# afermg/aliby

Measured on AMD Instinct MI355X. Metric: FOV tiles/sec (whole node), higher is better.
Workload: dtype u16 pixels, f64 feature accumulators, f32 dynamics, bfloat16 U-Net

## Files before the change

aliby_amd/csrc/nn_conv.hip:

```cpp
#include "common.h"
#include "conv_launch.h"
#include "conv_mfma.h"

namespace {

struct ConvArgs {
  const uint4* in;
  const uint4* wpk;
  uint4* out;
  uint4* pool;
  const float* scale;
  const float* shift;
  const float* bias;
  const uint4* res;
  int shift_stride, res_up;
  int cs, coff;
  int ocs, ocoff;
  int N, H, W;
  int G;
  int tiles_x, tiles_y, ntiles;
  int order;
  const uint4* pin;
  const uint4* pwpk;
  int pcs;
// ... 430 lines not shown
    if constexpr (PACK) {
      g0 = (tx * TW) / a.W;
      cst = tx * TW - g0 * a.W;
      half = (a.W - cst) >> 1;
    }
    const uint4* inN = a.in + (size_t)(PACK ? n * a.G : n) * IH * IW * a.cs + a.coff;
    int t0 = tid;
    asm volatile("" : "+v"(t0));
#pragma unroll
    for (int k = 0; k < GIT; ++k) {
      const int unit = t0 + k * 256;
      const int rpix = unit / NPL, oct = unit % NPL;
      const int rly = rpix / RLW, rlx = rpix - rly * RLW;
      const int iy = min(max(ry0 + rly, 0), IH - 1);
      int ix, img = 0;
      if constexpr (PACK) {
        const bool first = rlx <= half;
        ix = min(max(first ? (cst >> 1) - 1 + rlx : rlx - half - 1, 0), IW - 1);
        img = first ? g0 : min(g0 + 1, a.G - 1);
      } else {
        ix = min(max(rx0 + rlx, 0), IW - 1);
      }
      const uint4* g = inN + (unsigned)(((img * IH + iy) * IW + ix) * a.cs + oct);
      __builtin_amdgcn_global_load_lds((const __attribute__((address_space(1))) void*)g,
                                       (__attribute__((address_space(3))) void*)(ldsR + k * 256 + wave_u * 64), 16, 0, 0);
    }
  };

  if (walk.count > 0) issue_dma(walk.first);
  for (int stamp_tile = 0; stamp_tile < walk.count; ++stamp_tile) {
    const int tile = walk.first + stamp_tile * walk.step;
    CONV_STAMP(0);
    const int tx = tile % a.tiles_x, tyn = tile / a.tiles_x;
    const int ty = tyn % a.tiles_y, n = tyn / a.tiles_y;
    const int y0 = ty * TH, x0 = tx * TW;
    int g0 = 0, cst = x0, kb = 1 << 20, nimg = n;
    if constexpr (PACK) {
      g0 = x0 / a.W;
      cst = x0 - g0 * a.W;
      kb = a.W - cst;
      nimg = n * a.G;
    }
    const int second = (PACK && px >= kb) ? 1 : 0;
    const int gx = PACK ? (second ? px - kb : cst + px) : x0 + px;
    const int irow = PACK ? (g0 + second) * a.H : 0;

    f32x2_t sh[4], sh1[PACK ? 4 : 1];
    {
      const float* sp = a.shift + (size_t)(nimg + g0) * a.shift_stride + pl * 8;
#pragma unroll
      for (int k = 0; k < 4; ++k) sh[k] = f32x2_t{sp[2 * k], sp[2 * k + 1]};
      if constexpr (PACK) {
        const float* sq = a.shift + (size_t)(nimg + min(g0 + 1, a.G - 1)) * a.shift_stride + pl * 8;
#pragma unroll
        for (int k = 0; k < 4; ++k) sh1[k] = f32x2_t{sq[2 * k], sq[2 * k + 1]};
      }
    }
    float4 b4[4] = {};
    if (a.bias) {
      const float4* bp = reinterpret_cast<const float4*>(a.bias + c0);
#pragma unroll
      for (int q = 0; q < 4; ++q) b4[q] = bp[q];
    }
    uint4 rr[R][2];
    auto load_res = [&](int pass) { conv_load_res<R>(a, nimg, irow, y0 + (rg * PASSES + pass) * R, gx, c0, rr); };
    if (a.res) load_res(0);
    CONV_STAMP(1);
    asm volatile("s_waitcnt vmcnt(0)" ::: "memory");
    __syncthreads();
    CONV_STAMP(2);
    if constexpr (cfg::LOWA) {
      const int ry0 = (y0 >> 1) - 1, rx0 = (x0 >> 1) - 1;
      int p0 = pix0;
      asm volatile("" : "+v"(p0));
#pragma unroll
      for (int it = 0; it < ITERS; ++it) {
        const int rpix = p0 + it * PIX_PER_IT;
        const int rly = rpix / RLW, rlx = rpix - rly * RLW;
        const unsigned keep = 0u - (unsigned)((unsigned)(ry0 + rly) < (unsigned)IH && (unsigned)(rx0 + rlx) < (unsigned)IW);
        const uint4 o = conv_act8(ldsR[min(rpix, cfg::APIX - 1) * NPL + pl], sc, sh, keep);
        if (it == ITERS - 1 && rpix >= cfg::APIX) continue;
        ldsA[pl * PLANE + rpix] = o;
      }
    } else {
      const int ry0 = UP ? (y0 >> 1) - 1 : y0 - 1, rx0 = UP ? (x0 >> 1) - 1 : x0 - 1;
      int p0 = pix0, qy = ly0, qx = lx0;
      asm volatile("" : "+v"(p0), "+v"(qy), "+v"(qx));
#pragma unroll
      for (int it = 0; it < ITERS; ++it) {
        int lx = qx + (it * PIX_PER_IT) % LW, ly = qy + (it * PIX_PER_IT) / LW;
        if (lx >= LW) { lx -= LW; ly += 1; }
        const int gy = y0 - 1 + ly, gxi = x0 - 1 + lx;
        const int pix = p0 + it * PIX_PER_IT;
        unsigned keep;
        int rpix;
        uint4 o;
        if constexpr (PACK) {
          const int gapi = kb < 32 ? kb + 1 : TW + 2;
          const int bp = lx - 1 - (lx > gapi ? 1 : 0);
          const int snd = bp >= kb ? 1 : 0;
          const int c = snd ? bp - kb : cst + bp;
          keep = 0u - (unsigned)(lx != gapi && c >= 0 && c < a.W && !(bp == TW && kb == TW) && (unsigned)gy < (unsigned)a.H);
          const int rcol = snd ? (kb >> 1) + 1 + (c >> 1) : ((cst + bp) >> 1) - ((cst >> 1) - 1);
          rpix = min(max(((gy >> 1) - ry0) * RLW + rcol, 0), cfg::RLH * RLW - 1);
          f32x2_t shs[4];
#pragma unroll
          for (int k = 0; k < 4; ++k) shs[k] = snd ? sh1[k] : sh[k];
          o = conv_act8(ldsR[rpix * NPL + pl], sc, shs, keep);
        } else {
          keep = 0u - (unsigned)((unsigned)gy < (unsigned)a.H && (unsigned)gxi < (unsigned)a.W);
          rpix = UP ? min(((gy >> 1) - ry0) * RLW + ((gxi >> 1) - rx0), cfg::RLH * RLW - 1) : min(pix, RAW - 1);
          o = conv_act8(ldsR[rpix * NPL + pl], sc, sh, keep);
        }
        if (it == ITERS - 1 && pix >= RAW) continue;
        ldsA[pl * PLANE + pix] = o;
      }
    }
    CONV_STAMP(3);
    __syncthreads();
#pragma unroll
    for (int pass = 0; pass < PASSES; ++pass) {
      const int rbase = (rg * PASSES + pass) * R;
      f32x16_t acc[R];
      conv_seed<R>(acc, b4, rr, a.res != nullptr);
      __builtin_amdgcn_sched_barrier(0);
      if (pass == 0 && stamp_tile + 1 < walk.count) issue_dma(tile + walk.step);
      if (pass + 1 < PASSES && a.res) load_res(pass + 1);
      __builtin_amdgcn_sched_barrier(0);
      if (pass == 0) CONV_STAMP(4);
      if constexpr (cfg::LOWA) {
        const bf16x8_t* L0 = reinterpret_cast<const bf16x8_t*>(ldsA) + hh * PLANE + (rbase >> 1) * RLW + ((px + 1) >> 1);
        conv_mfma<R, KC, cfg::DEPTH, PLANE, RLW, true>(L0, wfrag, acc, L0 + 1 - (px & 1));
      } else {
        conv_mfma<R, KC, cfg::DEPTH, PLANE, LW>(reinterpret_cast<const bf16x8_t*>(ldsA) + hh * PLANE + rbase * LW + px + second, wfrag, acc);
      }
      if (pass == PASSES - 1) CONV_STAMP(5);
      conv_store<R>(a, nimg, irow, y0 + rbase, gx, c0, acc);
    }
    CONV_STAMP(6);
  }
}

struct PairBase {
  static constexpr int KC = 2, NPL = 4, R = 2, PASSES = 2;
  static constexpr int TH = 14, TWO = 30, MH = 16, MW = 32;
  static constexpr int RAW_MID = MH * MW, PLANE_MID = RAW_MID + (10 - RAW_MID % 8) % 8;
  static constexpr int MID_SLOTS = NPL * PLANE_MID + 8;
  static constexpr int DEPTH = 6;
};
struct PairCfg : PairBase {
  static constexpr int IH = 18, IW = 34;
  static constexpr int RAW_IN = IH * IW, PLANE_IN = RAW_IN + (10 - RAW_IN % 8) % 8;
  static constexpr int PIX_PER_IT = 256 / NPL, ITERS = (RAW_IN + PIX_PER_IT - 1) / PIX_PER_IT;
  static constexpr int SLOTS = NPL * PLANE_IN + 2 * MID_SLOTS;
  static constexpr int LDS_BYTES = SLOTS * 16;
};

template <bool POOL, bool HEAD>
__global__ __launch_bounds__(512, 1) void k_conv_pair32(ConvArgs a) {
  static_assert(!(POOL && HEAD), "either the pooled output (down block) or the output head (last unit)");
  using cfg = PairCfg;
  constexpr int KC = cfg::KC, NPL = cfg::NPL, R = cfg::R, PASSES = cfg::PASSES, TH = cfg::TH, TWO = cfg::TWO;
  constexpr int IW_ = cfg::IW, MW = cfg::MW, PLANE_IN = cfg::PLANE_IN, PLANE_MID = cfg::PLANE_MID, RAW_IN = cfg::RAW_IN;
  constexpr int PIX_PER_IT = cfg::PIX_PER_IT, ITERS = cfg::ITERS;
  extern __shared__ uint4 lds[];
  uint4* const ldsIn = lds;
  uint4* const ldsMid0 = lds + NPL * PLANE_IN;
  __shared__ __align__(16) float tabB[64];
  __shared__ __align__(16) float biasA[32];
  __shared__ float hconst[HEAD ? 2 * 32 + 4 : 1];

  const int consumer = threadIdx.x >> 8;
  const int tid = threadIdx.x & 255, lane = tid & 63, wave = tid >> 6;
  const int px = lane & 31, hh = lane >> 5;
  const int c0 = hh * 16;

  const TileWalk walk = tile_walk(a.ntiles, a.order);
  const int my_tiles = walk.count;

  if (!consumer) {
    bf16x8_t wA[9 * KC];
    {
      const bf16x8_t* pa = reinterpret_cast<const bf16x8_t*>(a.wpk) + lane;
#pragma unroll
      for (int i = 0; i < 9 * KC; ++i) wA[i] = pa[i * 64];
    }
    const int pl = tid % NPL, pix0 = tid / NPL;
    const int ly0 = pix0 / IW_, lx0 = pix0 - ly0 * IW_;
    f32x2_t sc[4];
#pragma unroll
    for (int k = 0; k < 4; ++k) sc[k] = f32x2_t{a.scale[pl * 8 + 2 * k], a.scale[pl * 8 + 2 * k + 1]};
    if (tid < 32) biasA[tid] = a.bias ? a.bias[tid] : 0.f;
    uint4 v[ITERS];
    unsigned inside = 0;
    auto request = [&](int tile) {
      const int tx = tile % a.tiles_x, tyn = tile / a.tiles_x;
      const int ty = tyn % a.tiles_y, n = tyn / a.tiles_y;
      const int y0 = ty * TH, x0 = tx * TWO;
      const uint4* inN = a.in + (size_t)n * a.H * a.W * a.cs + a.coff;
      inside = 0;
#pragma unroll
      for (int u = 0; u < ITERS; ++u) {
        int lx = lx0 + (u * PIX_PER_IT) % IW_, ly = ly0 + (u * PIX_PER_IT) / IW_;
        if (lx >= IW_) { lx -= IW_; ly += 1; }
        const int gy = y0 - 2 + ly, gxi = x0 - 2 + lx;
        inside |= (unsigned)((unsigned)gy < (unsigned)a.H && (unsigned)gxi < (unsigned)a.W) << u;
        const int cy = min(max(gy, 0), a.H - 1), cx = min(max(gxi, 0), a.W - 1);
        v[u] = inN[(unsigned)((cy * a.W + cx) * a.cs + pl)];
      }
    };
    if (my_tiles > 0) request(walk.first);
    for (int it = 0; it < my_tiles; ++it) {
      const int tile = walk.first + it * walk.step;
      const int tx = tile % a.tiles_x, tyn = tile / a.tiles_x;
      const int ty = tyn % a.tiles_y, n = tyn / a.tiles_y;
      const int y0 = ty * TH, x0 = tx * TWO;
      uint4* const ldsMid = ldsMid0 + (it & 1) * cfg::MID_SLOTS;
      f32x2_t sh[4];
      {
        const float* sp = a.shift + (size_t)n * a.shift_stride + pl * 8;
#pragma unroll
        for (int k = 0; k < 4; ++k) sh[k] = f32x2_t{sp[2 * k], sp[2 * k + 1]};
      }
      if (tid < 32) {
        tabB[tid] = a.scale2[tid];
        tabB[32 + tid] = a.shift2[(size_t)n * a.shift2_stride + tid];
      }
#pragma unroll
      for (int u = 0; u < ITERS; ++u) {
        const uint4 o = conv_act8(v[u], sc, sh, 0u - ((inside >> u) & 1u));
        if (u == ITERS - 1 && pix0 + u * PIX_PER_IT >= RAW_IN) continue;
        ldsIn[pl * PLANE_IN + pix0 + u * PIX_PER_IT] = o;
      }
      __syncthreads();
      if (it + 1 < my_tiles) request(tile + walk.step);
      __builtin_amdgcn_sched_barrier(0);
#pragma unroll
      for (int pass = 0; pass < PASSES; ++pass) {
        const int mbase = (wave * PASSES + pass) * R;
        f32x16_t acc[R];
        {
          float4 b4[4];
#pragma unroll
          for (int q = 0; q < 4; ++q) b4[q] = reinterpret_cast<const float4*>(biasA + c0)[q];
#pragma unroll
          for (int r = 0; r < R; ++r) acc_seed(acc[r], b4);
        }
        __builtin_amdgcn_sched_barrier(0);
        conv_mfma<R, KC, cfg::DEPTH, PLANE_IN, IW_>(reinterpret_cast<const bf16x8_t*>(ldsIn) + hh * PLANE_IN + mbase * IW_ + px, wA, acc);
        __builtin_amdgcn_sched_barrier(0);
        const int mgx = x0 - 1 + px;
#pragma unroll
        for (int r = 0; r < R; ++r) {
          const int mgy = y0 - 1 + mbase + r;
          const unsigned keep = 0u - (unsigned)((unsigned)mgy < (unsigned)a.H && (unsigned)mgx < (unsigned)a.W);
#pragma unroll
          for (int half = 0; half < 2; ++half) {
            f32x2_t s2[4], h2[4];
            const float4* tp = reinterpret_cast<const float4*>(tabB + c0 + 8 * half);
            const float4 sa = tp[0], sb = tp[1], ha = tp[8], hb = tp[9];
            s2[0] = f32x2_t{sa.x, sa.y}; s2[1] = f32x2_t{sa.z, sa.w}; s2[2] = f32x2_t{sb.x, sb.y}; s2[3] = f32x2_t{sb.z, sb.w};
            h2[0] = f32x2_t{ha.x, ha.y}; h2[1] = f32x2_t{ha.z, ha.w}; h2[2] = f32x2_t{hb.x, hb.y}; h2[3] = f32x2_t{hb.z, hb.w};
            const uint4 raw = make_uint4(cv_pack2(acc[r][8 * half + 0], acc[r][8 * half + 1]), cv_pack2(acc[r][8 * half + 2], acc[r][8 * half + 3]),
                                         cv_pack2(acc[r][8 * half + 4], acc[r][8 * half + 5]), cv_pack2(acc[r][8 * half + 6], acc[r][8 * half + 7]));
            ldsMid[(2 * hh + half) * PLANE_MID + (mbase + r) * MW + px] = conv_act8(raw, s2, h2, keep);
          }
        }
      }
      __syncthreads();
    }
    __syncthreads();
    __syncthreads();
  } else {
    bf16x8_t wB[9 * KC];
    {
      const bf16x8_t* pb = reinterpret_cast<const bf16x8_t*>(a.wpk2) + lane;
#pragma unroll
      for (int i = 0; i < 9 * KC; ++i) wB[i] = pb[i * 64];
    }
    HeadW hwf;
    if constexpr (HEAD) {
      hwf = head_weights(a.hw, a.hO, lane);
      if (tid < 32) {
        hconst[tid] = a.hscale[tid];
        hconst[32 + tid] = a.hshift[tid];
        if (tid < 4) hconst[64 + tid] = tid < a.hO ? a.hbias[tid] : 0.f;
      }
    }
    float4 b4[4];
    load_bias4(a.bias2, c0, b4);
    __syncthreads();
    __syncthreads();
    for (int it = 0; it < my_tiles; ++it) {
      const int tile = walk.first + it * walk.step;
      const int tx = tile % a.tiles_x, tyn = tile / a.tiles_x;
      const int ty = tyn % a.tiles_y, n = tyn / a.tiles_y;
      const int y0 = ty * TH, x0 = tx * TWO;
      const uint4* const ldsMid = ldsMid0 + (it & 1) * cfg::MID_SLOTS;
      const int gx = (px < TWO && x0 + px < a.W) ? x0 + px : a.W;
#pragma unroll
      for (int pass = 0; pass < PASSES; ++pass) {
        const int rbase = (wave * PASSES + pass) * R;
        if (rbase < TH) {
          uint4 rr[R][2];
          if (a.res) conv_load_res<R>(a, n, 0, y0 + rbase, min(gx, a.W - 1), c0, rr);
          f32x16_t acc[R];
          conv_seed<R>(acc, b4, rr, a.res != nullptr);
          __builtin_amdgcn_sched_barrier(0);
          conv_mfma<R, KC, cfg::DEPTH, PLANE_MID, MW>(reinterpret_cast<const bf16x8_t*>(ldsMid) + hh * PLANE_MID + rbase * MW + px, wB, acc);
          if constexpr (HEAD) {
#pragma unroll
            for (int r = 0; r < R; ++r) {
              const f32x16_t y = head_from_acc(acc[r], hconst, hconst + 32, hwf, hh);
              const int gy = y0 + rbase + r;
              if (hh == 0 && gx < a.W && gy < a.H) {
                float* hp = a.hout + (size_t)n * a.hO * a.H * a.W + (size_t)gy * a.W + gx;
                const float yo[4] = {y[0], y[1], y[2], y[3]};
                for (int o = 0; o < a.hO; ++o) hp[(size_t)o * a.H * a.W] = yo[o] + hconst[64 + o];
              }
            }
          }
          if (!HEAD || a.out) conv_store<R>(a, n, 0, y0 + rbase, gx, c0, acc);
          if constexpr (POOL) {
            const int PH = a.H >> 1, PW = a.W >> 1;
            const int gy = y0 + rbase;
            const bool writer = (px & 1) == 0 && gx + 1 < a.W && gy + 1 < a.H;
            uint4* pp = a.pool + (size_t)n * PH * PW * a.ocs + a.ocoff + (unsigned)(((gy >> 1) * PW + (min(gx, a.W - 1) >> 1)) * a.ocs + (c0 >> 3));
#pragma unroll
            for (int half = 0; half < 2; ++half) {
              unsigned pk[4];
#pragma unroll
              for (int q = 0; q < 4; ++q) {
                const float v0 = fmaxf(acc[0][half * 8 + 2 * q], acc[1][half * 8 + 2 * q]);
                const float v1 = fmaxf(acc[0][half * 8 + 2 * q + 1], acc[1][half * 8 + 2 * q + 1]);
                pk[q] = cv_pack2(fmaxf(v0, __shfl_xor(v0, 1)), fmaxf(v1, __shfl_xor(v1, 1)));
              }
              if (writer) pp[half] = make_uint4(pk[0], pk[1], pk[2], pk[3]);
            }
          }
        }
        __syncthreads();
      }
    }
  }
}

struct FirstPairCfg : PairBase {
  static constexpr int AH = 18, AW = 36;
  static constexpr int P0_WORDS = 2 * AH * AW;
  static constexpr int RAWP_WORDS = MH * MW;
  static constexpr int VALS = 2 * AH * AW, ITERS = (VALS + 255) / 256;
  static constexpr int LDS_BYTES = 2 * MID_SLOTS * 16 + P0_WORDS * 4 + 2 * RAWP_WORDS * 4;
};

__global__ __launch_bounds__(512, 1) void k_conv_first_pair(ConvArgs a) {
  using cfg = FirstPairCfg;
  constexpr int KC = cfg::KC, R = cfg::R, PASSES = cfg::PASSES, TH = cfg::TH, TWO = cfg::TWO, MW = cfg::MW;
  constexpr int AH = cfg::AH, AW = cfg::AW, PLANE_MID = cfg::PLANE_MID, ITERS = cfg::ITERS;
  extern __shared__ uint4 lds[];
  uint4* const ldsMid0 = lds;
  unsigned* const P0 = reinterpret_cast<unsigned*>(lds + 2 * cfg::MID_SLOTS);
  unsigned* const rawP0 = P0 + cfg::P0_WORDS;
  __shared__ __align__(16) float tabB[64];

  const int consumer = threadIdx.x >> 8;
  const int tid = threadIdx.x & 255, lane = tid & 63, wave = tid >> 6;
  const int px = lane & 31, hh = lane >> 5;
  const int c0 = hh * 16;

  const TileWalk walk = tile_walk(a.ntiles, a.order);
  const int my_tiles = walk.count;
  const size_t plane = (size_t)a.H * a.W;

  if (!consumer) {
    bf16x8_t wF[2];
    {
      const int m = lane & 31, co = conv_row_channel(m);
#pragma unroll
      for (int kc = 0; kc < 2; ++kc) {
        unsigned r4[4];
#pragma unroll
        for (int j2 = 0; j2 < 4; ++j2) {
          float v[2];
#pragma unroll
          for (int e = 0; e < 2; ++e) {
            const int k = 16 * kc + 8 * hh + 2 * j2 + e, c = k / 12, ty = (k % 12) / 4, tx = k % 4;
            v[e] = (c < a.fcin && tx < 3 && k < 24) ? a.fw[((size_t)co * a.fcin + c) * 9 + ty * 3 + tx] : 0.f;
          }
          r4[j2] = cv_pack2(v[0], v[1]);
        }
        wF[kc] = __builtin_bit_cast(bf16x8_t, make_uint4(r4[0], r4[1], r4[2], r4[3]));
      }
    }
    int goff[2][2];
    unsigned gmask[2][2];
#pragma unroll
    for (int kc = 0; kc < 2; ++kc)
#pragma unroll
      for (int g = 0; g < 2; ++g) {
        const int k = 16 * kc + 8 * hh + 4 * g;
        const bool live = k < 24 && k / 12 < a.fcin;
        goff[kc][g] = live ? (k / 12) * AH * AW + ((k % 12) / 4) * AW : 0;
        gmask[kc][g] = live ? 0xffffffffu : 0u;
      }
    if (tid < 32) {
      tabB[tid] = a.scale2[tid];
      tabB[32 + tid] = a.shift2[tid];
    }
    const float fs0 = a.fscale[0], fh0 = a.fshift[0];
    const float fs1 = a.fcin > 1 ? a.fscale[1] : 0.f, fh1 = a.fcin > 1 ? a.fshift[1] : 0.f;
    float v[ITERS];
    unsigned inside = 0;
    auto request = [&](int tile) {
      const int tx = tile % a.tiles_x, tyn = tile / a.tiles_x;
      const int ty = tyn % a.tiles_y, n = tyn / a.tiles_y;
      const int y0 = ty * TH, x0 = tx * TWO;
      inside = 0;
#pragma unroll
      for (int u = 0; u < ITERS; ++u) {
        const int i = tid + 256 * u;
        const int c = i / (AH * AW), rem = i - c * (AH * AW), r = rem / AW, q = rem - r * AW;
        const int gy = y0 - 2 + r, gx = x0 - 2 + q;
        const bool ok = i < cfg::VALS && c < a.fcin && (unsigned)gy < (unsigned)a.H && (unsigned)gx < (unsigned)a.W;
        inside |= (unsigned)ok << u;
        const int cy = min(max(gy, 0), a.H - 1), cx = min(max(gx, 0), a.W - 1), cc = min(c, a.fcin - 1);
        v[u] = a.fx[((size_t)n * a.fcin + cc) * plane + (size_t)cy * a.W + cx];
      }
    };
    if (my_tiles > 0) request(walk.first);
    unsigned short* const P0h = reinterpret_cast<unsigned short*>(P0);
    for (int it = 0; it < my_tiles; ++it) {
      const int tile = walk.first + it * walk.step;
      const int tx = tile % a.tiles_x, tyn = tile / a.tiles_x;
      const int ty = tyn % a.tiles_y;
      const int y0 = ty * TH, x0 = tx * TWO;
      uint4* const ldsMid = ldsMid0 + (it & 1) * cfg::MID_SLOTS;
      unsigned short* const rawPh = reinterpret_cast<unsigned short*>(rawP0 + (it & 1) * cfg::RAWP_WORDS);
#pragma unroll
      for (int u = 0; u < ITERS; ++u) {
        const int i = tid + 256 * u;
        if (i >= cfg::VALS) break;
        const int c = i / (AH * AW), rem = i - c * (AH * AW), r = rem / AW, q = rem - r * AW;
        const bool ok = (inside >> u) & 1u;
        const unsigned short b = (unsigned short)cv_f2bf(ok ? first_relu(v[u], c ? fs1 : fs0, c ? fh1 : fh0) : 0.f);
        P0h[2 * i] = b;
        if (q > 0) P0h[2 * (i - 1) + 1] = b;
        if (q == AW - 1) P0h[2 * i + 1] = 0;
        if (r >= 2 && q >= 2 && q < 2 + MW)
          rawPh[2 * ((r - 2) * MW + (q - 2)) + c] = (unsigned short)(cv_pack2(ok ? v[u] : 0.f, 0.f) & 0xffffu);
      }
      if (a.fcin < 2) {
        for (int i = tid; i < cfg::RAWP_WORDS; i += 256) rawPh[2 * i + 1] = 0;
      }
      __syncthreads();
      if (it + 1 < my_tiles) request(tile + walk.step);
      __builtin_amdgcn_sched_barrier(0);
#pragma unroll
      for (int pass = 0; pass < PASSES; ++pass) {
        const int mbase = (wave * PASSES + pass) * R;
        const int mgx = x0 - 1 + px;
#pragma unroll
        for (int r = 0; r < R; ++r) {
          const int m = mbase + r;
          f32x16_t acc;
#pragma unroll
          for (int k = 0; k < 16; ++k) acc[k] = 0.f;
#pragma unroll
          for (int kc = 0; kc < 2; ++kc) {
            const unsigned* w0 = P0 + goff[kc][0] + m * AW + px;
            const unsigned* w1 = P0 + goff[kc][1] + m * AW + px;
            const uint4 bfrag = make_uint4(w0[0] & gmask[kc][0], w0[2] & gmask[kc][0], w1[0] & gmask[kc][1], w1[2] & gmask[kc][1]);
            acc = __builtin_amdgcn_mfma_f32_32x32x16_bf16(wF[kc], __builtin_bit_cast(bf16x8_t, bfrag), acc, 0, 0, 0);
          }
          const int mgy = y0 - 1 + m;
          const unsigned keep = 0u - (unsigned)((unsigned)mgy < (unsigned)a.H && (unsigned)mgx < (unsigned)a.W);
#pragma unroll
          for (int half = 0; half < 2; ++half) {
            f32x2_t s2[4], h2[4];
            const float4* tp = reinterpret_cast<const float4*>(tabB + c0 + 8 * half);
            const float4 sa = tp[0], sb = tp[1], ha = tp[8], hb = tp[9];
            s2[0] = f32x2_t{sa.x, sa.y}; s2[1] = f32x2_t{sa.z, sa.w}; s2[2] = f32x2_t{sb.x, sb.y}; s2[3] = f32x2_t{sb.z, sb.w};
            h2[0] = f32x2_t{ha.x, ha.y}; h2[1] = f32x2_t{ha.z, ha.w}; h2[2] = f32x2_t{hb.x, hb.y}; h2[3] = f32x2_t{hb.z, hb.w};
            const uint4 raw = make_uint4(cv_pack2(acc[8 * half + 0], acc[8 * half + 1]), cv_pack2(acc[8 * half + 2], acc[8 * half + 3]),
                                         cv_pack2(acc[8 * half + 4], acc[8 * half + 5]), cv_pack2(acc[8 * half + 6], acc[8 * half + 7]));
            ldsMid[(2 * hh + half) * PLANE_MID + m * MW + px] = conv_act8(raw, s2, h2, keep);
          }
        }
      }
      __syncthreads();
    }
    __syncthreads();
    __syncthreads();
  } else {
    bf16x8_t wB[9 * KC];
// ... 114 lines not shown
  }
  if constexpr (COUT == 32 && CIN == 32 && !UP && !PACK) {
    ARG_CHECK(!a.pool && a.hO >= 1 && a.hO <= 3, "conv3x3: fused head: 1..3 output channels, no pooled output");
    return launch<k_conv3x3<CIN, COUT, UP, false, 0, TALL, false, true>, 256>(ctx, a, cfg::LDS_BYTES, CAP, stream);
  } else {
    aliby_set_error("conv3x3: the fused output head is built for the (32,32) unit only");
    return ALIBY_ERR_UNSUPPORTED;
  }
}

template <int CIN, int COUT, bool UP>
int launch_conv(aliby_ctx* ctx, ConvArgs& a, hipStream_t stream) {
  static const bool use_dma = env_int("ALIBY_CONV_DMA", UP) != 0;
  if (use_dma && !a.pool && !a.pin && !a.hout) {
    if constexpr (UP && COUT >= 64) {
      static const int pack_up = env_int("ALIBY_CONV_PACK", 7);
      if ((pack_up & 4) && (a.W == 56 || a.W == 112) && a.N % (224 / a.W) == 0 && a.H % DmaCfg<CIN, COUT, UP, true>::TH == 0)
        return launch_conv_dma<CIN, COUT, UP, true>(ctx, a, stream);
    }
    return launch_conv_dma<CIN, COUT, UP>(ctx, a, stream);
  }
  constexpr bool CAN_TALL = (CIN >= 64 && COUT >= 128) || (CIN == 32 && COUT == 32);
  if constexpr (!UP && COUT >= 64) {
    static const int pack_on = env_int("ALIBY_CONV_PACK", 7);
    if ((pack_on & (COUT >= 128 ? 1 : 2)) && !a.pin && (a.W == 28 || a.W == 56 || a.W == 112) && a.N % (224 / a.W) == 0 &&
        a.H % ConvCfg<CIN, COUT, false, true>::TH == 0) {
      if constexpr (CIN == 64 && COUT == 64) {
        static const bool tall64 = env_int("ALIBY_CONV_TALL64", 1) != 0;
        if (tall64 && a.H % ConvCfg<CIN, COUT, true, true>::TH == 0) return launch_conv_reg<CIN, COUT, UP, true, true>(ctx, a, stream);
      }
      return launch_conv_reg<CIN, COUT, UP, false, true>(ctx, a, stream);
    }
  }
  if (CAN_TALL && !a.pin && a.H % (2 * ConvCfg<CIN, COUT, false>::TH) == 0) return launch_conv_reg<CIN, COUT, UP, CAN_TALL>(ctx, a, stream);
  return launch_conv_reg<CIN, COUT, UP, false>(ctx, a, stream);
}

}

struct HeadArgs { const float *scale, *shift, *w, *bias; float* out; int channels; };

static int conv3x3_entry(aliby_ctx* ctx, const void* in, const void* wpk, void* out, const float* scale,
                         const float* shift, int shift_per_sample, const float* bias, const void* res,
                         int res_up, int N, int H, int W, int CIN, int COUT, int in_up,
                         int in_channels, int in_channel0, int out_channels, int out_channel0,
                         void* pool_out, const void* proj_in, const void* proj_wpk, int proj_channels, void* stream_,
                         const HeadArgs* head = nullptr) {
  hipStream_t stream = static_cast<hipStream_t>(stream_);
  ARG_CHECK(ctx && in && wpk && (out || head) && scale && shift, "conv3x3: null argument");
  ARG_CHECK(N > 0 && H > 0 && W > 0, "conv3x3: empty shape");
  ARG_CHECK(!in_up || ((H & 1) == 0 && (W & 1) == 0), "conv3x3: upsampled input needs even H, W");
  ARG_CHECK(!res || !res_up || ((H & 1) == 0 && (W & 1) == 0), "conv3x3: upsampled residual needs even H, W");
  ConvArgs a;
  a.in = static_cast<const uint4*>(in);
  a.wpk = static_cast<const uint4*>(wpk);
  a.out = static_cast<uint4*>(out);
  a.scale = scale;
  a.shift = shift;
  a.bias = bias;
  a.res = static_cast<const uint4*>(res);
  a.shift_stride = shift_per_sample == 1 ? CIN : shift_per_sample;
  a.res_up = res_up ? 1 : 0;
  a.pool = static_cast<uint4*>(pool_out);
  ARG_CHECK(!pool_out || ((H & 1) == 0 && (W & 1) == 0), "conv3x3: pooled output needs even H, W");
  if (in_channels <= 0) in_channels = CIN;
  ARG_CHECK(in_channels % 8 == 0 && in_channel0 % 8 == 0 && in_channel0 >= 0 && in_channel0 + CIN <= in_channels,
            "conv3x3: channel slice must be octet aligned and inside the input tensor");
  if (out_channels <= 0) out_channels = COUT;
  ARG_CHECK(out_channels % 8 == 0 && out_channel0 % 8 == 0 && out_channel0 >= 0 && out_channel0 + COUT <= out_channels,
            "conv3x3: output channel slice must be octet aligned and inside the output tensor");
  a.ocs = out_channels / 8;
  a.ocoff = out_channel0 / 8;
  a.trace = g_conv_trace;
  a.hscale = head ? head->scale : nullptr;
  a.hshift = head ? head->shift : nullptr;
  a.hw = head ? head->w : nullptr;
  a.hbias = head ? head->bias : nullptr;
  a.hout = head ? head->out : nullptr;
  a.hO = head ? head->channels : 0;
  a.pin = static_cast<const uint4*>(proj_in);
  a.pwpk = static_cast<const uint4*>(proj_wpk);
  a.pcs = proj_channels / 8;
  ARG_CHECK(!proj_in || (proj_wpk && proj_channels > 0 && proj_channels % 8 == 0), "conv3x3: fused projection needs packed weights and an octet-aligned width");
  a.cs = in_channels / 8;
  a.coff = in_channel0 / 8;
  a.N = N; a.H = H; a.W = W;
  if (CIN == 32 && COUT == 32 && !in_up) return launch_conv<32, 32, false>(ctx, a, stream);
  if (CIN == 64 && COUT == 32 && in_up) return launch_conv<64, 32, true>(ctx, a, stream);
  if (CIN == 64 && COUT == 64 && !in_up) return launch_conv<64, 64, false>(ctx, a, stream);
  if (CIN == 64 && COUT == 64 && in_up) return launch_conv<64, 64, true>(ctx, a, stream);
  if (CIN == 64 && COUT == 128) return in_up ? launch_conv<64, 128, true>(ctx, a, stream) : launch_conv<64, 128, false>(ctx, a, stream);
  if (CIN == 32 && COUT == 64 && !in_up) return launch_conv<32, 64, false>(ctx, a, stream);
  aliby_set_error("conv3x3: unsupported (CIN=%d, COUT=%d, upsample=%d) combination", CIN, COUT, in_up);
  return ALIBY_ERR_UNSUPPORTED;
}

extern "C" int aliby_nn_conv3x3_bf16(aliby_ctx* ctx, const void* in, const void* wpk, void* out, const float* scale,
                                     const float* shift, int shift_per_sample, const float* bias, const void* res,
                                     int res_up, int N, int H, int W, int CIN, int COUT, int in_up,
                                     int in_channels, int in_channel0, int out_channels, int out_channel0,
                                     void* pool_out, void* stream) {
  return conv3x3_entry(ctx, in, wpk, out, scale, shift, shift_per_sample, bias, res, res_up, N, H, W, CIN, COUT, in_up, in_channels,
                       in_channel0, out_channels, out_channel0, pool_out, nullptr, nullptr, 0, stream);
}

extern "C" int aliby_nn_conv3x3_proj_bf16(aliby_ctx* ctx, const void* in, const void* wpk, void* out, const float* scale,
                                          const float* shift, int shift_per_sample, const float* bias, int N, int H, int W,
                                          int CIN, int COUT, const void* proj_in, const void* proj_wpk, int proj_channels,
                                          void* stream) {
  ARG_CHECK(proj_in && proj_wpk, "conv3x3_proj: NULL projection operand");
  return conv3x3_entry(ctx, in, wpk, out, scale, shift, shift_per_sample, bias, nullptr, 0, N, H, W, CIN, COUT, 0, 0, 0, 0, 0, nullptr,
                       proj_in, proj_wpk, proj_channels, stream);
}

extern "C" int aliby_nn_conv3x3_head_bf16(aliby_ctx* ctx, const void* in, const void* wpk, void* out_or_null, const float* scale,
                                          const float* shift, int shift_per_sample, const float* bias, const void* res, int res_up,
                                          int N, int H, int W, int CIN, int COUT, const float* head_scale, const float* head_shift,
                                          const float* head_w, const float* head_bias, int head_channels, float* head_out,
                                          void* stream) {
  ARG_CHECK(head_scale && head_shift && head_w && head_bias && head_out, "conv3x3_head: NULL head operand");
  ARG_CHECK(CIN == 32 && COUT == 32, "conv3x3_head: built for the 32 -> 32 unit");
  const HeadArgs head = {head_scale, head_shift, head_w, head_bias, head_out, head_channels};
  return conv3x3_entry(ctx, in, wpk, out_or_null, scale, shift, shift_per_sample, bias, res, res_up, N, H, W, CIN, COUT, 0, 0, 0, 0, 0,
                       nullptr, nullptr, nullptr, 0, stream, &head);
}

extern "C" int aliby_nn_conv3x3_pair_bf16(aliby_ctx* ctx, const void* in, const void* wpk_a, const void* wpk_b, void* out_or_null,
                                          const float* scale_a, const float* shift_a, int shift_a_per_sample, const float* bias_a,
                                          const float* scale_b, const float* shift_b, int shift_b_per_sample, const float* bias_b,
                                          const void* res, int N, int H, int W, void* pool_out, const float* head_scale,
                                          const float* head_shift, const float* head_w, const float* head_bias, int head_channels,
                                          float* head_out, void* stream_) {
  hipStream_t stream = static_cast<hipStream_t>(stream_);
  ARG_CHECK(ctx && in && wpk_a && wpk_b && (out_or_null || head_out) && scale_a && shift_a && scale_b && shift_b, "conv3x3_pair: null argument");
  ARG_CHECK(N > 0 && H > 0 && W > 0, "conv3x3_pair: empty shape");
  ARG_CHECK(!pool_out || ((H & 1) == 0 && (W & 1) == 0), "conv3x3_pair: pooled output needs even H, W");
  ARG_CHECK(!head_out || (head_scale && head_shift && head_w && head_bias && head_channels >= 1 && head_channels <= 3 && !pool_out),
            "conv3x3_pair: the fused head needs its operands, 1..3 channels and no pooled output");
  ARG_CHECK(!pool_out || out_or_null, "conv3x3_pair: the pooled output comes with the full output");
  ConvArgs a = {};
  a.in = static_cast<const uint4*>(in);
  a.wpk = static_cast<const uint4*>(wpk_a);
  a.wpk2 = static_cast<const uint4*>(wpk_b);
  a.out = static_cast<uint4*>(out_or_null);
  a.pool = static_cast<uint4*>(pool_out);
  a.scale = scale_a; a.shift = shift_a; a.bias = bias_a;
  a.scale2 = scale_b; a.shift2 = shift_b; a.bias2 = bias_b;
  a.shift_stride = shift_a_per_sample == 1 ? 32 : shift_a_per_sample;
  a.shift2_stride = shift_b_per_sample == 1 ? 32 : shift_b_per_sample;
  a.res = static_cast<const uint4*>(res);
  a.res_up = 0;
  a.cs = 4; a.coff = 0; a.ocs = 4; a.ocoff = 0;
  a.N = N; a.H = H; a.W = W; a.G = 1;
  a.hscale = head_scale; a.hshift = head_shift; a.hw = head_w; a.hbias = head_bias; a.hout = head_out; a.hO = head_out ? head_channels : 0;
  a.tiles_x = (W + PairCfg::TWO - 1) / PairCfg::TWO;
  a.tiles_y = (H + PairCfg::TH - 1) / PairCfg::TH;
  const long long nt = (long long)N * a.tiles_x * a.tiles_y;
  ARG_CHECK(nt < INT_MAX, "conv3x3_pair: too many tiles");
  a.ntiles = (int)nt;
  constexpr int CAP = 32;
  if (!head_out && !pool_out) return launch<k_conv_pair32<false, false>, 512>(ctx, a, PairCfg::LDS_BYTES, CAP, stream);
  if (!head_out) return launch<k_conv_pair32<true, false>, 512>(ctx, a, PairCfg::LDS_BYTES, CAP, stream);
  return launch<k_conv_pair32<false, true>, 512>(ctx, a, PairCfg::LDS_BYTES, CAP, stream);
}

extern "C" int aliby_nn_first_pair_bf16(aliby_ctx* ctx, const float* tiles, int N, int Cin, int H, int W, const float* scale0,
                                        const float* shift0, const float* w_oihw, const void* wpk1, const float* scale1,
                                        const float* shift1, const float* bias1, const void* proj_wpk, void* out, void* stream_) {
  hipStream_t stream = static_cast<hipStream_t>(stream_);
  ARG_CHECK(ctx && tiles && scale0 && shift0 && w_oihw && wpk1 && scale1 && shift1 && bias1 && proj_wpk && out, "first_pair: null argument");
  ARG_CHECK(N > 0 && H > 0 && W > 0 && Cin >= 1 && Cin <= 2, "first_pair: Cin must be 1 or 2");
  ConvArgs a = {};
  a.fx = tiles; a.fw = w_oihw; a.fscale = scale0; a.fshift = shift0; a.fcin = Cin;
  a.wpk2 = static_cast<const uint4*>(wpk1);
  a.scale2 = scale1; a.shift2 = shift1; a.bias2 = bias1; a.shift2_stride = 0;
  a.pwpk = static_cast<const uint4*>(proj_wpk);
  a.out = static_cast<uint4*>(out);
  a.cs = 4; a.coff = 0; a.ocs = 4; a.ocoff = 0;
  a.N = N; a.H = H; a.W = W; a.G = 1;
  a.tiles_x = (W + FirstPairCfg::TWO - 1) / FirstPairCfg::TWO;
  a.tiles_y = (H + FirstPairCfg::TH - 1) / FirstPairCfg::TH;
  const long long nt = (long long)N * a.tiles_x * a.tiles_y;
  ARG_CHECK(nt < INT_MAX, "first_pair: too many tiles");
  a.ntiles = (int)nt;
  return launch<k_conv_first_pair, 512>(ctx, a, FirstPairCfg::LDS_BYTES, 32, stream);
}

extern "C" int aliby_nn_out_head_bf16(aliby_ctx* ctx, const void* x, const float* scale, const float* shift, const float* w,
                                      const float* bias, int N, int H, int W, int C, int O, float* out, void* stream) {
  ARG_CHECK(ctx && x && scale && shift && w && bias && out, "out_head: null argument");
  ARG_CHECK(C == 32 && O >= 1 && O <= 4, "out_head: C must be 32 and 1 <= O <= 4");
  ARG_CHECK(N > 0 && H > 0 && W > 0, "out_head: empty shape");
  const size_t P = (size_t)H * W, total = (size_t)N * P;
  const size_t waves = (total + 31) / 32;
  const unsigned blocks = (unsigned)((waves + 3) / 4 < 4096 ? (waves + 3) / 4 : 4096);
  hipLaunchKernelGGL(k_out_head_mfma, dim3(blocks), dim3(256), 0, static_cast<hipStream_t>(stream), static_cast<const uint4*>(x), scale, shift, w,
                     bias, O, (size_t)N, P, out);
  KERNEL_CHECK();
  return ALIBY_OK;
}

extern "C" int aliby_debug_conv_trace(aliby_ctx* ctx, void* stamps_dev) {
  ARG_CHECK(ctx != nullptr, "ctx is NULL");
  g_conv_trace = static_cast<unsigned long long*>(stamps_dev);
  return ALIBY_OK;
}

static int pack_entry(aliby_ctx* ctx, const float* w, int COUT, int CIN_src, int CIN, int taps, void* wpk, void* stream_) {
  hipStream_t stream = static_cast<hipStream_t>(stream_);
  ARG_CHECK(ctx && w && wpk, "pack_conv: null argument");
  ARG_CHECK(COUT > 0 && COUT % 32 == 0 && CIN % 16 == 0 && CIN_src > 0 && CIN_src <= CIN, "pack_conv: COUT must be a multiple of 32 and CIN of 16");
  const size_t total = (size_t)COUT * CIN * taps;
  hipLaunchKernelGGL(k_pack_conv3x3, dim3((unsigned)((total + 255) / 256)), dim3(256), 0, stream, w, COUT, CIN_src, CIN, taps,
                     static_cast<unsigned short*>(wpk), total);
  KERNEL_CHECK();
  return ALIBY_OK;
}

extern "C" int aliby_nn_pack_conv3x3_bf16(aliby_ctx* ctx, const float* w_oihw, int COUT, int CIN_src, int CIN, void* wpk, void* stream) {
  return pack_entry(ctx, w_oihw, COUT, CIN_src, CIN, 9, wpk, stream);
}

extern "C" int aliby_nn_pack_conv1x1_bf16(aliby_ctx* ctx, const float* w_oi, int COUT, int CIN_src, int CIN, void* wpk, void* stream) {
  return pack_entry(ctx, w_oi, COUT, CIN_src, CIN, 1, wpk, stream);
}
```

Before: 631.9.

## Split pair-conv into half-tile rounds so unit B overlaps unit A

Restructures the producer/consumer pair kernel into finer-grained rounds. The input window and scale/shift table are now double-buffered. Unit A computes intermediate rows 0-7 of tile t while unit B processes the low rows of tile t-1, then A does rows 8-15 while B finishes rows 6-13. The aim is to keep both wave groups busy instead of serialising full tiles between barriers, at the cost of more LDS, more barriers per tile and more complex row-dependency invariants. Trace stamps are also wired in.

```diff
diff --git a/aliby_amd/csrc/nn_conv.hip b/aliby_amd/csrc/nn_conv.hip
--- a/aliby_amd/csrc/nn_conv.hip
+++ b/aliby_amd/csrc/nn_conv.hip
@@ -606,21 +606,33 @@
   static constexpr int IH = 18, IW = 34;
   static constexpr int RAW_IN = IH * IW, PLANE_IN = RAW_IN + (10 - RAW_IN % 8) % 8;
   static constexpr int PIX_PER_IT = 256 / NPL, ITERS = (RAW_IN + PIX_PER_IT - 1) / PIX_PER_IT;
-  static constexpr int SLOTS = NPL * PLANE_IN + 2 * MID_SLOTS;
+  static constexpr int IN_SLOTS = NPL * PLANE_IN;
+  static constexpr int SLOTS = 2 * IN_SLOTS + 2 * MID_SLOTS;
   static constexpr int LDS_BYTES = SLOTS * 16;
+  static constexpr int a_row(int wave, int pass) { return 8 * pass + R * wave; }
+  static constexpr int b_row(int wave, int high) { return high ? 6 + R * wave : R * wave; }
+  static constexpr int B_LOW_WAVES = 3;
 };
+static_assert(PairCfg::a_row(3, 0) + PairCfg::R == 8 && PairCfg::a_row(3, 1) + PairCfg::R == PairCfg::MH, "unit A: rows 0-7 in the first pass, 8-15 in the second");
+static_assert(PairCfg::b_row(PairCfg::B_LOW_WAVES - 1, 0) + PairCfg::R + 2 <= 8, "unit B's low pass reads intermediate rows 0-7 only (written one interval earlier)");
+static_assert(PairCfg::b_row(PairCfg::B_LOW_WAVES - 1, 0) + PairCfg::R == PairCfg::b_row(0, 1) && PairCfg::b_row(3, 1) + PairCfg::R == PairCfg::TH, "unit B: rows 0-5, then 6-13");
+static_assert(PairCfg::b_row(3, 1) + PairCfg::R + 2 <= PairCfg::MH, "unit B's high pass stays inside the intermediate tile");
+static_assert(PairCfg::a_row(1, 1) % 2 == 0 && PairCfg::b_row(1, 0) % 2 == 0 && PairCfg::b_row(1, 1) % 2 == 0 && PairCfg::TH % 2 == 0, "row pairs are even-aligned (pooled epilogue)");
+static_assert(PairCfg::LDS_BYTES + 1024 <= 160 * 1024, "two windows, two sets of planes and the static tables fit the CU's LDS");
+
+__host__ __device__ constexpr int pair_barriers(int my_tiles) { return 2 * my_tiles + 2; }
 
 template <bool POOL, bool HEAD>
 __global__ __launch_bounds__(512, 1) void k_conv_pair32(ConvArgs a) {
   static_assert(!(POOL && HEAD), "either the pooled output (down block) or the output head (last unit)");
   using cfg = PairCfg;
-  constexpr int KC = cfg::KC, NPL = cfg::NPL, R = cfg::R, PASSES = cfg::PASSES, TH = cfg::TH, TWO = cfg::TWO;
+  constexpr int KC = cfg::KC, NPL = cfg::NPL, R = cfg::R, TH = cfg::TH, TWO = cfg::TWO;
   constexpr int IW_ = cfg::IW, MW = cfg::MW, PLANE_IN = cfg::PLANE_IN, PLANE_MID = cfg::PLANE_MID, RAW_IN = cfg::RAW_IN;
   constexpr int PIX_PER_IT = cfg::PIX_PER_IT, ITERS = cfg::ITERS;
   extern __shared__ uint4 lds[];
-  uint4* const ldsIn = lds;
-  uint4* const ldsMid0 = lds + NPL * PLANE_IN;
-  __shared__ __align__(16) float tabB[64];
+  uint4* const ldsIn0 = lds;
+  uint4* const ldsMid0 = lds + 2 * cfg::IN_SLOTS;
+  __shared__ __align__(16) float tabB[2][64];
   __shared__ __align__(16) float biasA[32];
   __shared__ float hconst[HEAD ? 2 * 32 + 4 : 1];
 
@@ -631,6 +643,7 @@
 
   const TileWalk walk = tile_walk(a.ntiles, a.order);
   const int my_tiles = walk.count;
+  const int rounds = pair_barriers(my_tiles) / 2;
 
   if (!consumer) {
     bf16x8_t wA[9 * KC];
@@ -646,30 +659,31 @@
     for (int k = 0; k < 4; ++k) sc[k] = f32x2_t{a.scale[pl * 8 + 2 * k], a.scale[pl * 8 + 2 * k + 1]};
     if (tid < 32) biasA[tid] = a.bias ? a.bias[tid] : 0.f;
     uint4 v[ITERS];
-    unsigned inside = 0;
+    auto window_pixel = [&](int u, int y0, int x0, int& gy, int& gxi) {
+      int lx = lx0 + (u * PIX_PER_IT) % IW_, ly = ly0 + (u * PIX_PER_IT) / IW_;
+      if (lx >= IW_) { lx -= IW_; ly += 1; }
+      gy = y0 - 2 + ly;
+      gxi = x0 - 2 + lx;
+      return (unsigned)gy < (unsigned)a.H && (unsigned)gxi < (unsigned)a.W;
+    };
     auto request = [&](int tile) {
       const int tx = tile % a.tiles_x, tyn = tile / a.tiles_x;
       const int ty = tyn % a.tiles_y, n = tyn / a.tiles_y;
-      const int y0 = ty * TH, x0 = tx * TWO;
       const uint4* inN = a.in + (size_t)n * a.H * a.W * a.cs + a.coff;
-      inside = 0;
 #pragma unroll
       for (int u = 0; u < ITERS; ++u) {
-        int lx = lx0 + (u * PIX_PER_IT) % IW_, ly = ly0 + (u * PIX_PER_IT) / IW_;
-        if (lx >= IW_) { lx -= IW_; ly += 1; }
-        const int gy = y0 - 2 + ly, gxi = x0 - 2 + lx;
-        inside |= (unsigned)((unsigned)gy < (unsigned)a.H && (unsigned)gxi < (unsigned)a.W) << u;
+        int gy, gxi;
+        window_pixel(u, ty * TH, tx * TWO, gy, gxi);
         const int cy = min(max(gy, 0), a.H - 1), cx = min(max(gxi, 0), a.W - 1);
         v[u] = inN[(unsigned)((cy * a.W + cx) * a.cs + pl)];
       }
     };
-    if (my_tiles > 0) request(walk.first);
-    for (int it = 0; it < my_tiles; ++it) {
+    auto activate = [&](auto parc, int it) {
+      constexpr int par = decltype(parc)::value;
       const int tile = walk.first + it * walk.step;
       const int tx = tile % a.tiles_x, tyn = tile / a.tiles_x;
       const int ty = tyn % a.tiles_y, n = tyn / a.tiles_y;
-      const int y0 = ty * TH, x0 = tx * TWO;
-      uint4* const ldsMid = ldsMid0 + (it & 1) * cfg::MID_SLOTS;
+      uint4* const ldsIn = ldsIn0 + par * cfg::IN_SLOTS;
       f32x2_t sh[4];
       {
         const float* sp = a.shift + (size_t)n * a.shift_stride + pl * 8;
@@ -677,54 +691,81 @@
         for (int k = 0; k < 4; ++k) sh[k] = f32x2_t{sp[2 * k], sp[2 * k + 1]};
       }
       if (tid < 32) {
-        tabB[tid] = a.scale2[tid];
-        tabB[32 + tid] = a.shift2[(size_t)n * a.shift2_stride + tid];
+        tabB[par][tid] = a.scale2[tid];
+        tabB[par][32 + tid] = a.shift2[(size_t)n * a.shift2_stride + tid];
       }
 #pragma unroll
       for (int u = 0; u < ITERS; ++u) {
-        const uint4 o = conv_act8(v[u], sc, sh, 0u - ((inside >> u) & 1u));
+        int gy, gxi;
+        const uint4 o = conv_act8(v[u], sc, sh, 0u - (unsigned)window_pixel(u, ty * TH, tx * TWO, gy, gxi));
         if (u == ITERS - 1 && pix0 + u * PIX_PER_IT >= RAW_IN) continue;
         ldsIn[pl * PLANE_IN + pix0 + u * PIX_PER_IT] = o;
       }
+    };
+    auto unit_a = [&](auto passc, auto parc, int it) {
+      constexpr int pass = decltype(passc)::value, par = decltype(parc)::value;
+      const int tile = walk.first + it * walk.step;
+      const int tx = tile % a.tiles_x, tyn = tile / a.tiles_x;
+      const int ty = tyn % a.tiles_y;
+      const int y0 = ty * TH, x0 = tx * TWO;
+      const uint4* const ldsIn = ldsIn0 + par * cfg::IN_SLOTS;
+      uint4* const ldsMid = ldsMid0 + par * cfg::MID_SLOTS;
+      const float* const tab = tabB[par];
+      const int mbase = cfg::a_row(wave, pass);
+      f32x16_t acc[R];
+      {
+        float4 b4[4];
+#pragma unroll
+        for (int q = 0; q < 4; ++q) b4[q] = reinterpret_cast<const float4*>(biasA + c0)[q];
+#pragma unroll
+        for (int r = 0; r < R; ++r) acc_seed(acc[r], b4);
+      }
+      __builtin_amdgcn_sched_barrier(0);
+      conv_mfma<R, KC, cfg::DEPTH, PLANE_IN, IW_>(reinterpret_cast<const bf16x8_t*>(ldsIn) + hh * PLANE_IN + mbase * IW_ + px, wA, acc);
+      __builtin_amdgcn_sched_barrier(0);
+      const int mgx = x0 - 1 + px;
+#pragma unroll
+      for (int r = 0; r < R; ++r) {
+        const int mgy = y0 - 1 + mbase + r;
+        const unsigned keep = 0u - (unsigned)((unsigned)mgy < (unsigned)a.H && (unsigned)mgx < (unsigned)a.W);
+#pragma unroll
+        for (int half = 0; half < 2; ++half) {
+          f32x2_t s2[4], h2[4];
+          const float4* tp = reinterpret_cast<const float4*>(tab + c0 + 8 * half);
+          const float4 sa = tp[0], sb = tp[1], ha = tp[8], hb = tp[9];
+          s2[0] = f32x2_t{sa.x, sa.y}; s2[1] = f32x2_t{sa.z, sa.w}; s2[2] = f32x2_t{sb.x, sb.y}; s2[3] = f32x2_t{sb.z, sb.w};
+          h2[0] = f32x2_t{ha.x, ha.y}; h2[1] = f32x2_t{ha.z, ha.w}; h2[2] = f32x2_t{hb.x, hb.y}; h2[3] = f32x2_t{hb.z, hb.w};
+          const uint4 raw = make_uint4(cv_pack2(acc[r][8 * half + 0], acc[r][8 * half + 1]), cv_pack2(acc[r][8 * half + 2], acc[r][8 * half + 3]),
+                                       cv_pack2(acc[r][8 * half + 4], acc[r][8 * half + 5]), cv_pack2(acc[r][8 * half + 6], acc[r][8 * half + 7]));
+          ldsMid[(2 * hh + half) * PLANE_MID + (mbase + r) * MW + px] = conv_act8(raw, s2, h2, keep);
+        }
+      }
+    };
+    if (my_tiles > 0) request(walk.first);
+    __builtin_amdgcn_s_waitcnt(0x0F70);
+    __builtin_amdgcn_sched_barrier(0);
+    auto round = [&](auto parc, int t) {
+      constexpr int par = decltype(parc)::value;
+      const int stamp_tile = t;
+      if (t > 0) unit_a(std::integral_constant<int, 1>{}, std::integral_constant<int, 1 - par>{}, t - 1);
+      __builtin_amdgcn_sched_barrier(0);
+      if (t < my_tiles) activate(parc, t);
+      CONV_STAMP(0);
       __syncthreads();
-      if (it + 1 < my_tiles) request(tile + walk.step);
-      __builtin_amdgcn_sched_barrier(0);
-#pragma unroll
-      for (int pass = 0; pass < PASSES; ++pass) {
-        const int mbase = (wave * PASSES + pass) * R;
-        f32x16_t acc[R];
-        {
-          float4 b4[4];
-#pragma unroll
-          for (int q = 0; q < 4; ++q) b4[q] = reinterpret_cast<const float4*>(biasA + c0)[q];
-#pragma unroll
-          for (int r = 0; r < R; ++r) acc_seed(acc[r], b4);
-        }
+      CONV_STAMP(1);
+      if (t < my_tiles) {
+        if (t + 1 < my_tiles) request(walk.first + (t + 1) * walk.step);
         __builtin_amdgcn_sched_barrier(0);
-        conv_mfma<R, KC, cfg::DEPTH, PLANE_IN, IW_>(reinterpret_cast<const bf16x8_t*>(ldsIn) + hh * PLANE_IN + mbase * IW_ + px, wA, acc);
-        __builtin_amdgcn_sched_barrier(0);
-        const int mgx = x0 - 1 + px;
-#pragma unroll
-        for (int r = 0; r < R; ++r) {
-          const int mgy = y0 - 1 + mbase + r;
-          const unsigned keep = 0u - (unsigned)((unsigned)mgy < (unsigned)a.H && (unsigned)mgx < (unsigned)a.W);
-#pragma unroll
-          for (int half = 0; half < 2; ++half) {
-            f32x2_t s2[4], h2[4];
-            const float4* tp = reinterpret_cast<const float4*>(tabB + c0 + 8 * half);
-            const float4 sa = tp[0], sb = tp[1], ha = tp[8], hb = tp[9];
-            s2[0] = f32x2_t{sa.x, sa.y}; s2[1] = f32x2_t{sa.z, sa.w}; s2[2] = f32x2_t{sb.x, sb.y}; s2[3] = f32x2_t{sb.z, sb.w};
-            h2[0] = f32x2_t{ha.x, ha.y}; h2[1] = f32x2_t{ha.z, ha.w}; h2[2] = f32x2_t{hb.x, hb.y}; h2[3] = f32x2_t{hb.z, hb.w};
-            const uint4 raw = make_uint4(cv_pack2(acc[r][8 * half + 0], acc[r][8 * half + 1]), cv_pack2(acc[r][8 * half + 2], acc[r][8 * half + 3]),
-                                         cv_pack2(acc[r][8 * half + 4], acc[r][8 * half + 5]), cv_pack2(acc[r][8 * half + 6], acc[r][8 * half + 7]));
-            ldsMid[(2 * hh + half) * PLANE_MID + (mbase + r) * MW + px] = conv_act8(raw, s2, h2, keep);
-          }
-        }
-      }
+        unit_a(std::integral_constant<int, 0>{}, parc, t);
+      }
+      CONV_STAMP(2);
       __syncthreads();
-    }
-    __syncthreads();
-    __syncthreads();
+      CONV_STAMP(3);
+    };
+    for (int t = 0; t < rounds; t += 2) {
+      round(std::integral_constant<int, 0>{}, t);
+      if (t + 1 < rounds) round(std::integral_constant<int, 1>{}, t + 1);
+    }
   } else {
     bf16x8_t wB[9 * KC];
     {
@@ -743,19 +784,19 @@
     }
     float4 b4[4];
     load_bias4(a.bias2, c0, b4);
-    __syncthreads();
-    __syncthreads();
-    for (int it = 0; it < my_tiles; ++it) {
+    for (int t = 0; t < rounds; ++t) {
+      const int it = t - 1;
       const int tile = walk.first + it * walk.step;
       const int tx = tile % a.tiles_x, tyn = tile / a.tiles_x;
       const int ty = tyn % a.tiles_y, n = tyn / a.tiles_y;
       const int y0 = ty * TH, x0 = tx * TWO;
       const uint4* const ldsMid = ldsMid0 + (it & 1) * cfg::MID_SLOTS;
+      const int stamp_tile = t;
       const int gx = (px < TWO && x0 + px < a.W) ? x0 + px : a.W;
 #pragma unroll
-      for (int pass = 0; pass < PASSES; ++pass) {
-        const int rbase = (wave * PASSES + pass) * R;
-        if (rbase < TH) {
+      for (int pass = 0; pass < 2; ++pass) {
+        const int rbase = cfg::b_row(wave, pass);
+        if (it >= 0 && (pass == 1 || wave < cfg::B_LOW_WAVES)) {
           uint4 rr[R][2];
           if (a.res) conv_load_res<R>(a, n, 0, y0 + rbase, min(gx, a.W - 1), c0, rr);
           f32x16_t acc[R];
@@ -793,7 +834,9 @@
             }
           }
         }
+        CONV_STAMP(4 + 2 * pass);
         __syncthreads();
+        CONV_STAMP(5 + 2 * pass);
       }
     }
   }
@@ -1214,6 +1257,7 @@
   a.res_up = 0;
   a.cs = 4; a.coff = 0; a.ocs = 4; a.ocoff = 0;
   a.N = N; a.H = H; a.W = W; a.G = 1;
+  a.trace = g_conv_trace;
   a.hscale = head_scale; a.hshift = head_shift; a.hw = head_w; a.hbias = head_bias; a.hout = head_out; a.hO = head_out ? head_channels : 0;
   a.tiles_x = (W + PairCfg::TWO - 1) / PairCfg::TWO;
   a.tiles_y = (H + PairCfg::TH - 1) / PairCfg::TH;
```

Result: no change. 630.4 (-0.3%).
